# fxzjshm/simple-radio-telescope-backend

Hardware: AMD Instinct MI355X
Metric: baseband Msamples/sec/node + real-time ratio, J1644-4559 config at 1/2/4/8 MI355X (higher is better)
Workload: dtype fp32; 1 GPU; model=J1644-4559 coherent-dedispersion single-pulse pipeline, baseband_input_count=1073741824, nsamps_reserved=23494656, baseband_input_bits=2, spectrum_channel_count=2048, rfi=True, phase_table=False, fft_backend=native, parallelism=stream-sharded dp1, global_batch=1, seq_len=1073741824

## Files before the change

csrc/bind/module.cpp:

```cpp

#include <torch/extension.h>
#include <pybind11/numpy.h>
#include <ATen/cuda/CUDAContext.h>
#include <c10/cuda/CUDAGuard.h>

#include <functional>
#include <vector>

#include "../engine/engine.h"
#include "../fft/native_fft.h"
#include "../include/srtb_kernels.h"

namespace {

using namespace srtb_hip;

hipStream_t cur_stream() {
  return at::cuda::getCurrentCUDAStream().stream();
}

void check(hipError_t e, const char* what) { check_hip(e, what); }

#define CHECK_CUDA(t) TORCH_CHECK((t).is_cuda(), #t " must be on GPU")
#define CHECK_CONTIG(t) TORCH_CHECK((t).is_contiguous(), #t " must be contiguous")
// ... 627 lines not shown
  auto out = torch::empty({nc}, torch::TensorOptions()
                                    .dtype(torch::kComplexFloat)
                                    .device(dev));
  check(dedisp_poly_factors(cptr(out), (size_t)nc, (uint32_t)n,
                            (size_t)stride, f_min, f_c, df, dm, cur_stream()),
        "dedisp_poly_factors");
  return out;
}

torch::Tensor t_native_rfft(torch::Tensor x) {
  CHECK_CUDA(x);
  CHECK_CONTIG(x);
  TORCH_CHECK(x.scalar_type() == torch::kFloat32);
  const size_t n = x.numel();
  const size_t m = n / 2;
  auto stream = cur_stream();
  NativeFft plan;
  plan.plan(m, 1, -1, stream);
  auto z = torch::empty({(int64_t)m},
                        x.options().dtype(torch::kComplexFloat));
  auto packed = x.view({(int64_t)m, 2});
  auto work = torch::empty_like(z);
  work.copy_(torch::view_as_complex(packed));
  plan.exec(cptr(work), cptr(z), stream);
  check(r2c_post_process(cptr(z), cptr(z), m, nullptr, nullptr, stream),
        "r2c post");
  check(hipStreamSynchronize(stream), "native_rfft sync");
  return z;
}


double time_iters(hipStream_t stream, int iters, const std::function<void()>& f) {
  hipEvent_t e0, e1;
  check(hipEventCreate(&e0), "ev");
  check(hipEventCreate(&e1), "ev");
  f();
  check(hipStreamSynchronize(stream), "warm sync");
  check(hipEventRecord(e0, stream), "rec");
  for (int i = 0; i < iters; ++i) f();
  check(hipEventRecord(e1, stream), "rec");
  check(hipEventSynchronize(e1), "sync");
  float ms = 0;
  check(hipEventElapsedTime(&ms, e0, e1), "elapsed");
  hipEventDestroy(e0);
  hipEventDestroy(e1);
  return ms / iters;
}

double t_bench_fft(int64_t len, int64_t batch, int64_t sign, int64_t iters,
                   std::string backend) {
  auto stream = cur_stream();
// ... 20 lines not shown
    ms = time_iters(stream, (int)iters, [&] {
      hipfftExecC2C(h, reinterpret_cast<hipfftComplex*>(xp),
                    reinterpret_cast<hipfftComplex*>(yp),
                    sign < 0 ? HIPFFT_FORWARD : HIPFFT_BACKWARD);
    });
    hipfftDestroy(h);
  }
  return ms;
}

double t_bench_rfft(int64_t n, int64_t iters, std::string backend) {
  auto stream = cur_stream();
  auto x = torch::randn({n}, torch::TensorOptions()
                                 .dtype(torch::kFloat32)
                                 .device(torch::kCUDA));
  auto y = torch::empty({n / 2 + 1, 2}, x.options());
  float* xp = x.data_ptr<float>();
  float2* yp = reinterpret_cast<float2*>(y.data_ptr());
  double ms = 0;
  if (backend == "native") {
    const size_t m = n / 2;
    NativeFft plan;
    plan.plan(m, 1, -1, stream);
    ms = time_iters(stream, (int)iters, [&] {
      plan.exec(reinterpret_cast<float2*>(xp), yp, stream);
      check(r2c_post_process(yp, yp, m, nullptr, nullptr, stream), "post");
    });
  } else {
    hipfftHandle h;
    check_fft(hipfftCreate(&h), "create");
    long long n1[1] = {(long long)n};
    size_t ws = 0;
    check_fft(hipfftMakePlanMany64(h, 1, n1, nullptr, 1, 0, nullptr, 1, 0,
                                   HIPFFT_R2C, 1, &ws),
              "plan");
    check_fft(hipfftSetStream(h, stream), "stream");
    ms = time_iters(stream, (int)iters, [&] {
      hipfftExecR2C(h, xp, reinterpret_cast<hipfftComplex*>(yp));
    });
    hipfftDestroy(h);
  }
  return ms;
}


class PyEngine {
 public:
  PyEngine(int64_t n, int64_t nbits, int64_t channels, double freq_low,
           double bandwidth, double sample_rate, double dm,
// ... 310 lines not shown
  m.def("subtract_mean", &t_subtract_mean);
  m.def("count_signal", &t_count_signal);
  m.def("inclusive_scan", &t_inclusive_scan);
  m.def("boxcar", &t_boxcar);
  m.def("boxcar_ladder", &t_boxcar_ladder, py::arg("cumsum"),
        py::arg("lengths"), py::arg("snr"));
  m.def("resample_power", &t_resample_power);
  m.def("normalize_by_mean", &t_normalize_by_mean);
  m.def("generate_pixmap", &t_generate_pixmap);
  m.def("running_mean", &t_running_mean);
  m.def("correlate", &t_correlate);
  m.def("filterbank_detect", &t_filterbank_detect, py::arg("wf"),
        py::arg("flags"), py::arg("valid_rows"), py::arg("tscrunch"),
        py::arg("fscrunch"), py::arg("reverse"));
  m.def("filterbank_channel_stats", &t_filterbank_channel_stats, py::arg("P"));
  m.def("filterbank_quantize", &t_filterbank_quantize, py::arg("P"),
        py::arg("mean"), py::arg("std"));
  m.def("fold_block", &t_fold_block, py::arg("wf"), py::arg("flags"),
        py::arg("valid"), py::arg("nbin"), py::arg("phi"), py::arg("dphi"),
        py::arg("acc"), py::arg("hits"), py::arg("weights"));
  m.def("native_fft", &t_native_fft, py::arg("x"), py::arg("sign"));
  m.def("native_fft_sk", &t_native_fft_sk, py::arg("x"));
  m.def("native_rfft", &t_native_rfft, py::arg("x"));
  m.def("preop_backward_fft", &t_preop_backward_fft, py::arg("spec"),
        py::arg("maxcol_log2"), py::arg("final_log2"), py::arg("f_min"),
        py::arg("f_c"), py::arg("df"), py::arg("dms"),
        py::arg("ranges") = std::vector<std::vector<int64_t>>{},
        py::arg("enable_rfi") = false, py::arg("threshold") = 0.0,
        py::arg("channel_count") = 1);
  m.def("dedisp_poly_factors", &t_dedisp_poly_factors);
  m.def("bench_fft", &t_bench_fft, py::arg("len"), py::arg("batch"),
        py::arg("sign"), py::arg("iters") = 20, py::arg("backend") = "native");
  m.def("bench_rfft", &t_bench_rfft, py::arg("n"), py::arg("iters") = 20,
        py::arg("backend") = "native");

  py::class_<PyEngine>(m, "PipelineEngine")
      .def(py::init<int64_t, int64_t, int64_t, double, double, double, double,
                    double, double, double, int64_t, int64_t,
                    std::vector<std::vector<int64_t>>, bool, bool, bool,
                    int64_t, int64_t, int64_t, bool, int64_t, int64_t,
                    int64_t, int64_t, int64_t, double, double, double>(),
           py::arg("n"), py::arg("nbits"), py::arg("channels"),
           py::arg("freq_low"), py::arg("bandwidth"), py::arg("sample_rate"),
           py::arg("dm"), py::arg("rfi_threshold") = 10.0,
           py::arg("sk_threshold") = 1.1, py::arg("snr_threshold") = 6.0,
           py::arg("max_boxcar") = 1024, py::arg("nsamps_reserved") = 0,
// ... 49 lines not shown
```

csrc/engine/engine.cpp:

```cpp
#include "engine.h"

#include <roctracer/roctx.h>

#include <algorithm>
#include <cmath>
#include <cstdlib>
#include <cstring>
#include <stdexcept>
#include <string>

namespace srtb_hip {

namespace {
constexpr double kD = 4.148808e3;

uint64_t fold_turns_to_word(double x) {
  const double v = std::ldexp(x, 64);
  if (v >= 0x1p64) return 0;
  if (v >= 0x1p63) return (uint64_t)v;
  return (uint64_t)std::llrint(v);
}

struct RoctxRange {
  bool on;
// ... 207 lines not shown
      check_hip(hipMalloc(&s.fold_table,
                          fold_table_words(fold_v_) * sizeof(uint32_t)),
                "fold table alloc");
      check_hip(hipHostMalloc(&s.h_fold_words, 2 * sizeof(uint64_t)),
                "pinned fold words");
      check_hip(hipMemset(s.fold_acc, 0, s_ * nb * sizeof(double)),
                "fold acc clear");
      check_hip(hipMemset(s.fold_hits, 0, nb * sizeof(uint64_t)),
                "fold hits clear");
      check_hip(hipMemset(s.fold_weights, 0, s_ * sizeof(uint64_t)),
                "fold weights clear");
      check_hip(hipDeviceSynchronize(), "fold clear sync");
    }
    fused_unpack_off_ = std::getenv("SRTB_NO_FUSED_UNPACK") != nullptr;
    if (const char* sc = std::getenv("SRTB_SERIAL_CHAINS"))
      serial_chains_ = std::atoi(sc) != 0 ? 1 : 0;
    const int be = cfg.fft_backend;
    native_fft_ = (be == 0 || be == 2) && NativeFft::supported(nc_);
    native_bwd_ = native_fft_ && NativeFft::supported(l_) &&
                  (be == 0 || l_ >= (1ull << 17));
    fuse_r2c_ = false;
    if (native_fft_) {
      s.nfwd.plan(nc_, 1, -1, s.stream);
      if (native_bwd_) {
        const char* b32 = std::getenv("SRTB_FFT_BWD32");
        if (b32 && std::atoi(b32) != 0)
          s.nbwd.plan(l_, s_, +1, s.stream, 5,
                      8);
        else
          s.nbwd.plan(l_, s_, +1, s.stream);
        const int wpr = s.nbwd.dif_sk_wgs_per_row();
        if (cfg.enable_sk && wpr > 0 && cfg.window_kind == 0)
          check_hip(hipMalloc(&s.sk_dif_partials,
                              s_ * (size_t)wpr * sizeof(float2)),
                    "sk dif partials");
      } else {
        s.plans.create_c2c_only(l_, s_, s.stream);
      }
      check_hip(hipStreamSynchronize(s.stream), "fft table sync");
      {
        const char* fe = std::getenv("SRTB_FUSE_R2C");
        const bool want = fe && std::atoi(fe) != 0;
        const int fwgs = s.nfwd.dif_sk_wgs_per_row();
        fuse_r2c_ = want && native_bwd_ && s.nbwd.first_pass_fusable() &&
                    fwgs > 0;
        if (fuse_r2c_) {
// ... 22 lines not shown
  if (cfg.use_phase_table) {
    check_hip(hipMalloc(&phase_table_, nc_ * sizeof(float2)), "table alloc");
    check_hip(dedisp_phase_table(phase_table_, nc_, f_min_, f_c_, df_, cfg.dm,
                                 slots_[0]->stream),
              "phase table");
    check_hip(hipStreamSynchronize(slots_[0]->stream), "table sync");
  }
}

PipelineEngine::~PipelineEngine() {
  for (auto& sp : slots_) {
    if (sp->stream) (void)hipStreamSynchronize(sp->stream);
  }
  for (auto& sp : slots_) {
    Slot& s = *sp;
    s.plans.destroy();
    (void)hipFree(s.raw);
    (void)hipFree(s.samples);
    (void)hipFree(s.spec);
    (void)hipFree(s.s2s4);
    if (s.sk_dif_partials) (void)hipFree(s.sk_dif_partials);
    if (s.xbuf) (void)hipFree(s.xbuf);
    if (s.fwd_pw) (void)hipFree(s.fwd_pw);
    (void)hipFree(s.flags);
    (void)hipFree(s.ts);
    (void)hipFree(s.ts_partial);
    (void)hipFree(s.cumsum);
    (void)hipFree(s.box);
    (void)hipFree(s.scan_scratch);
    (void)hipFree(s.partials);
    if (s.box_partials) (void)hipFree(s.box_partials);
    (void)hipFree(s.mean_power);
    (void)hipFree(s.sums);
    (void)hipFree(s.counters);
    (void)hipFree(s.thresholds);
    (void)hipHostFree(s.h_counters);
    (void)hipHostFree(s.h_thresholds);
    if (s.trial_w) {
      (void)hipFree(s.trial_w);
      (void)hipFree(s.trial_plane);
      (void)hipFree(s.trial_counters);
      (void)hipFree(s.trial_thresholds);
      (void)hipFree(s.trial_peak_val);
      (void)hipFree(s.trial_peak_idx);
      (void)hipHostFree(s.h_trial_counters);
      (void)hipHostFree(s.h_trial_thresholds);
// ... 208 lines not shown
                           (in_bits == 1 || in_bits == 2 || in_bits == 4 ||
                            in_bits == 8 || in_bits == -8 ||
                            in_bits == 16 || in_bits == -16) &&
                           !window_ && slots_[0]->nfwd.first_pass_fusable();
  if (dev_raw && !fuse_unpack) {
    check_hip(unpack(dev_raw, s.samples, n_, cfg_.baseband_input_bits,
                     window_, st),
              "unpack");
  } else if (!dev_raw && native_fft_) {
    check_hip(hipMemcpyAsync(s.samples, dev_samples, n_ * sizeof(float),
                             hipMemcpyDeviceToDevice, st),
              "samples d2d");
  } else if (!dev_raw) {
    fft_in = dev_samples;
  }
  if (native_fft_ && fr2c) {
    s.nfwd.exec(reinterpret_cast<float2*>(s.samples), s.spec, st,
                nullptr, cfg_.enable_rfi_s1 ? s.fwd_pw : nullptr,
                fuse_unpack ? dev_raw : nullptr, in_bits);
    if (cfg_.enable_rfi_s1)
      check_hip(r2c_mean_from_power(s.fwd_pw, fwd_pw_n_, s.spec, nc_,
                                    s.mean_power, st),
                "r2c mean");
  } else if (native_fft_) {
    s.nfwd.exec(reinterpret_cast<float2*>(s.samples), s.spec, st,
                nullptr, nullptr, fuse_unpack ? dev_raw : nullptr, in_bits);
    check_hip(r2c_post_process(
                  s.spec, s.spec, nc_,
                  cfg_.enable_rfi_s1 ? s.partials : nullptr,
                  cfg_.enable_rfi_s1 ? s.mean_power : nullptr, st),
              "r2c post");
  } else {
    s.plans.exec_r2c(const_cast<float*>(fft_in), s.spec);
    if (cfg_.enable_rfi_s1)
      check_hip(mean_power(s.spec, nc_, s.partials, s.mean_power, st),
                "meanp");
  }
}

void PipelineEngine::enqueue_back(Slot& s, double dm, const ResultRow& row,
                                  float* ts_dst, bool keep_spectrum) {
  hipStream_t st = s.stream;
  const float2* table = phase_table_;
  const bool fr2c = fuse_r2c_;
  const bool fuse_into_bwd = native_bwd_ && s.nbwd.first_pass_fusable();
  const FftPreop pre = make_preop(s, dm);
// ... 429 lines not shown
```

csrc/engine/engine.h:

```cpp

#pragma once

#include <hip/hip_runtime.h>

#include <array>
#include <cstdint>
#include <memory>
#include <vector>

#include "../fft/fft_plans.h"
#include "../fft/native_fft.h"
#include "../include/srtb_kernels.h"

namespace srtb_hip {

struct EngineConfig {
  size_t baseband_input_count = 1ull << 28;
  int baseband_input_bits = 8;
  size_t spectrum_channel_count = 1ull << 15;
  double freq_low = 1000.0;
  double bandwidth = 500.0;
  double sample_rate = 1e9;
  double dm = 0.0;
  float rfi_threshold = 10.0f;
// ... 158 lines not shown
  int n_slots_ = 2;

  float2* phase_table_ = nullptr;
  float* window_ = nullptr;
  float* watfft_window_ = nullptr;
  bool native_fft_ = false;
  bool fused_unpack_off_ = false;
  bool native_bwd_ = false;
  bool fuse_r2c_ = false;
  size_t fwd_pw_n_ = 0;


  struct Slot {
    hipStream_t stream = nullptr;
    hipEvent_t done = nullptr;
    bool busy = false;
    bool wf_zap_pending = false;
    float2* wf = nullptr;
    uint8_t* raw = nullptr;
    float* samples = nullptr;
    float2* spec = nullptr;
    float2* xbuf = nullptr;
    float2* fwd_pw = nullptr;
    float2* s2s4 = nullptr;
    float2* sk_dif_partials = nullptr;
    uint8_t* flags = nullptr;
    float* ts = nullptr;
    float* ts_partial = nullptr;
    float* cumsum = nullptr;
    float* box = nullptr;
    float* scan_scratch = nullptr;
    double* partials = nullptr;
    double* box_partials = nullptr;
    double* mean_power = nullptr;
    double* sums = nullptr;
    unsigned* counters = nullptr;
    float* thresholds = nullptr;
    unsigned* h_counters = nullptr;
    float* h_thresholds = nullptr;
    FftPlanSet plans;
    NativeFft nfwd, nbwd;
    hipGraphExec_t graph_exec = nullptr;
    const void* graph_host_src = nullptr;
    int graph_pending = 0;
    float2* trial_w = nullptr;
    float* trial_plane = nullptr;
// ... 34 lines not shown
```

csrc/fft/native_fft.h:

```cpp

#pragma once

#include <algorithm>
#include <cstdint>
#include <cstdlib>
#include <cmath>
#include <stdexcept>
#include <string>
#include <vector>

#include "../include/srtb_kernels.h"
#include "fft_plans.h"

namespace srtb_hip {

class NativeFft {
 public:
  static constexpr uint32_t kMaxPassLen = 4096;
  static int elems_per_wg() {
    const char* e = std::getenv("SRTB_FFT_ELEMS");
    int v = e ? std::atoi(e) : 4096;
    if (v < 512) v = 512;
    if (v > 8192) v = 8192;
    return v;
  }

  static bool is_pow2(size_t v) { return v && (v & (v - 1)) == 0; }

  static bool supported(size_t len) {
    return is_pow2(len) && len >= 2 &&
           len <= (size_t)kMaxPassLen * kMaxPassLen * kMaxPassLen;
  }

  NativeFft() = default;
  NativeFft(const NativeFft&) = delete;
  NativeFft& operator=(const NativeFft&) = delete;
  ~NativeFft() { destroy(); }

  void plan(size_t len, size_t batch, int sign, hipStream_t stream,
            int maxcol_log2_ovr = 0, int final_log2_ovr = 0) {
    destroy();
    if (!supported(len)) throw std::runtime_error("NativeFft: unsupported len");
    len_ = len;
    batch_ = batch;
    sign_ = sign;

    const size_t L = len;
    const int t = ilog2z(len);
    passes_.clear();
    if (t <= 12) {
      const char* we = std::getenv("SRTB_FFT_WAVE");
      const int wv = we ? std::atoi(we) : 1;
      if (t >= 8 && t <= 11 && wv != 0) {
        ensure_len_table((uint32_t)len, sign, stream);
        Pass p;
        p.kind = PassKind::kWave;
        p.d.n = (uint32_t)len;
        p.n_ffts = batch;
        p.tw_n = len_table((uint32_t)len);
        passes_.push_back(p);
        return;
      }
      if (t == 12 && !std::getenv("SRTB_FFT_NOSP_DIF")) {
        ensure_len_table((uint32_t)len, sign, stream);
        Pass p;
        p.kind = PassKind::kDif;
        p.d.n = (uint32_t)len;
        p.dif.n = (uint32_t)len;
// ... 99 lines not shown
      p.n_ffts = batch * (L / f[j]);
      p.tw_n = len_table(f[j]);
      p.tw_hi = mod_hi(M[j]);
      p.tw_lo = mod_lo(M[j]);
      passes_.push_back(p);
    }
    {
      const uint32_t fn = f[m - 1];
      ensure_len_table(fn, sign, stream);
      Pass p;
      p.kind = PassKind::kDif;
      p.d.n = fn;
      p.dif.n = fn;
      p.dif.out_c2 = L;
      p.dif.out_elem_coef = Cp[m - 1];
      p.dif.n_prefix = m - 1;
      for (int w = 0; w < m - 1; ++w) {
        p.dif.pf_bits[w] = ilog2z(f[w]);
        p.dif.pf_coef[w] = M[w + 1] / fn;
      }
      p.n_ffts = batch * (L / fn);
      p.tw_n = len_table(fn);
      passes_.push_back(p);
    }
  }

  int n_passes() const { return (int)passes_.size(); }

  bool first_pass_fusable() const {
    return !passes_.empty() && passes_[0].kind == PassKind::kCol;
  }

  bool preop_uses_poly(const FftPreop& preop) const {
    return first_pass_fusable() &&
           fft_col_preop_uses_poly(passes_[0].d, passes_[0].n_ffts, sign_,
                                   preop);
  }

  int dif_sk_wgs_per_row() const {
    if (passes_.empty() || passes_.back().kind != PassKind::kDif) return 0;
    const Pass& p = passes_.back();
    const size_t per_row = (len_ / p.dif.n);
    const int F = dif_f(p);
    if (per_row % F != 0) return 0;
    return (int)(per_row / F);
  }

  void exec(const float2* in, float2* out, hipStream_t stream,
            const FftPreop* preop = nullptr,
            float2* dif_sk_partials = nullptr,
            const uint8_t* decode2_raw = nullptr, int decode_bits = 2,
            float2* first_pass_out = nullptr) {
    if (passes_.empty()) throw std::runtime_error("NativeFft: not planned");
    if (passes_.size() > 1 && in == out && !first_pass_out)
      throw std::runtime_error("NativeFft: multi-pass needs out != in");
    if (preop && preop->r2c_m && !first_pass_out)
      throw std::runtime_error("NativeFft: r2c fusion needs first_pass_out");
    if (preop && !first_pass_fusable())
      throw std::runtime_error("NativeFft: preop needs a column first pass");
    if (decode2_raw && (preop || !first_pass_fusable()))
      throw std::runtime_error("NativeFft: decode2 needs a column first pass");
    float2* cur = const_cast<float2*>(in);
    for (size_t i = 0; i < passes_.size(); ++i) {
      Pass& p = passes_[i];
      const bool last = (i + 1 == passes_.size());
      float2* dst = last ? out : cur;
      const FftPreop* pre = (i == 0) ? preop : nullptr;
      switch (p.kind) {
        case PassKind::kStockham: {
          const int F = pick_f(p.d.n, p, p.n_ffts);
          check_hip(fft_stockham_pass(cur, dst, p.d, p.n_ffts, F,
                                      p.load_ffast, p.store_ffast, sign_,
                                      p.tw_n, p.tw_hi, p.tw_lo, stream),
                    "fft_stockham_pass");
          break;
        }
        case PassKind::kCol: {
          float2* o = (i == 0 && first_pass_out) ? first_pass_out : cur;
          check_hip(fft_col_pass(cur, o, p.d, p.n_ffts, sign_, p.tw_n,
                                 p.tw_hi, p.tw_lo, stream, pre,
                                 i == 0 ? decode2_raw : nullptr, decode_bits),
                    "fft_col_pass");
          dst = o;
          break;
        }
        case PassKind::kMid:
          check_hip(fft_mid512_pass(cur, cur, p.d, p.n_ffts, sign_, p.tw_n,
                                    stream),
                    "fft_mid512_pass");
          dst = cur;
          break;
        case PassKind::kWave:
          check_hip(fft_wave_pass(cur, dst, p.d.n, p.n_ffts, sign_, p.tw_n,
                                  stream),
                    "fft_wave_pass");
          break;
        case PassKind::kDif: {
          const int F = dif_f(p);
          check_hip(fft_dif_final(cur, dst, p.dif, p.n_ffts, F, sign_,
                                  p.tw_n, dif_sk_partials, stream),
                    "fft_dif_final");
          break;
        }
      }
      cur = dst;
    }
  }

  void destroy() {
    for (auto& t : tables_) (void)hipFree(t.ptr);
    tables_.clear();
    passes_.clear();
  }

 private:
  enum class PassKind { kStockham, kCol, kMid, kDif, kWave };

  struct Pass {
    PassKind kind = PassKind::kStockham;
    FftPassDesc d{};
// ... 8 lines not shown
  struct Table {
    int kind;
    size_t key;
    float2* ptr;
  };

  static int ilog2z(size_t v) {
    int t = 0;
    while ((1ull << t) < v) ++t;
    return t;
  }

  int dif_f(const Pass& p) const {
    int F = (p.dif.n <= 64) ? 32 : 16;
    if (const char* e = std::getenv("SRTB_FFT_DIF_F")) {
      const int v = std::atoi(e);
      if (v >= 1 && v <= 64 && (v & (v - 1)) == 0) F = v;
    }
    while (F > 1 &&
           ((size_t)p.dif.n + (size_t)F * (p.dif.n + 2)) * sizeof(float2) >
               80 * 1024)
      F >>= 1;
    while (F > 1 && p.n_ffts % F != 0) F >>= 1;
    return F;
  }

  int pick_f(uint32_t n, const Pass& p, size_t n_ffts) const {
    size_t f = (size_t)elems_per_wg() / n;
    if (f < 1) f = 1;
    while (f > 1 &&
           ((size_t)n + 2ull * f * (n + 2) + 16) * sizeof(float2) >
               160 * 1024)
      f >>= 1;
    while (f > 1 && n_ffts % f != 0) f >>= 1;
    if (p.d.d0 > 1 && f > p.d.d0) f = p.d.d0;
    while (f > 1 && n_ffts % f != 0) f >>= 1;
    return (int)f;
  }

  void ensure_len_table(uint32_t n, int sign, hipStream_t stream) {
    if (len_table(n)) return;
    float2* t = nullptr;
    check_hip(hipMalloc(&t, std::max<size_t>(n, 1) * sizeof(float2)),
              "tw_n alloc");
    check_hip(fft_build_twiddle(t, std::max<size_t>(n, 1), (double)n, sign,
                                stream),
// ... 22 lines not shown
    tables_.push_back({1, mod, thi});
    tables_.push_back({2, mod, tlo});
  }

  float2* len_table(uint32_t n) const {
    for (auto& t : tables_)
      if (t.kind == 0 && t.key == n) return t.ptr;
    return nullptr;
  }
  float2* mod_hi(size_t mod) const {
    for (auto& t : tables_)
      if (t.kind == 1 && t.key == mod) return t.ptr;
    return nullptr;
  }
  float2* mod_lo(size_t mod) const {
    for (auto& t : tables_)
      if (t.kind == 2 && t.key == mod) return t.ptr;
    return nullptr;
  }
  int mod_lo_bits(size_t mod) const { return mod_lo_bits_for(mod); }

  size_t len_ = 0, batch_ = 0;
  int sign_ = -1;
  std::vector<Pass> passes_;
  std::vector<Table> tables_;
};

}
```

csrc/include/srtb_kernels.h:

```cpp

#pragma once

#include <hip/hip_runtime.h>
#include <cstddef>
#include <cstdint>

namespace srtb_hip {

hipError_t unpack(const uint8_t* in, float* out, size_t out_count, int nbits,
                  const float* window, hipStream_t stream);

hipError_t unpack_interleaved_2pol(const int8_t* in, float* out0, float* out1,
                                   size_t count_per_pol, const float* window,
                                   hipStream_t stream);

hipError_t unpack_naocpsr_snap1(const int8_t* in, float* out0, float* out1,
                                size_t count_per_pol, const float* window,
                                hipStream_t stream);

hipError_t unpack_gznupsr_a1(const uint8_t* in, float* out0, float* out1,
                             float* out2, float* out3, int n_streams,
                             size_t count_per_stream, const float* window,
                             hipStream_t stream);

// ... 164 lines not shown
bool fft_col_preop_uses_poly(const FftPassDesc& d, size_t n_ffts, int sign,
                             const FftPreop& preop);

hipError_t dedisp_poly_factors(float2* out, size_t nc, uint32_t n,
                               size_t stride, double f_min, double f_c,
                               double df, double dm, hipStream_t stream);

struct DifFinalDesc {
  uint32_t n;
  unsigned long long out_c2;
  unsigned long long out_elem_coef;
  int n_prefix = 0;
  int pf_bits[4] = {0, 0, 0, 0};
  unsigned long long pf_coef[4] = {0, 0, 0, 0};
};
hipError_t fft_mid512_pass(const float2* in, float2* out,
                           const FftPassDesc& d, size_t n_ffts, int sign,
                           const float2* tw_n, hipStream_t stream);

hipError_t fft_dif_final(const float2* in, float2* out, const DifFinalDesc& d,
                         size_t n_ffts, int F, int sign, const float2* tw_n,
                         float2* sk_partials, hipStream_t stream);

hipError_t sk_combine_partials(const float2* partials, size_t rows,
                               int wgs_per_row, float2* s2s4,
                               hipStream_t stream);

hipError_t r2c_post_process(const float2* z, float2* x, size_t m,
                            double* mean_partials, double* out_mean,
                            hipStream_t stream);

hipError_t resample_power_2d(const float2* wf, size_t rows, size_t len,
                             float* out, int out_h, int out_w,
                             hipStream_t stream);

hipError_t normalize_by_mean(float* img, size_t n, const double* sum,
                             hipStream_t stream);

hipError_t generate_pixmap(const float* intensity, uint32_t* out, size_t n,
                           uint32_t color0, uint32_t color1,
                           uint32_t color_overflow, hipStream_t stream);

hipError_t running_mean_init(const float* data, size_t nsamp, size_t nchan,
                             size_t windowsize, float* ave, hipStream_t stream);
hipError_t running_mean(const float* data, size_t nsamp, size_t nchan,
                        uint8_t* out, size_t windowsize, float* ave,
// ... 11 lines not shown
```

csrc/kernels/fft.hip:

```cpp

#include <cmath>
#include <cstdlib>
#include "common.h"
#include "../include/srtb_kernels.h"

namespace srtb_hip {

namespace {

__device__ inline float2 cmulf(float2 a, float2 b) {
  return make_float2(a.x * b.x - a.y * b.y, a.x * b.y + a.y * b.x);
}

}

struct FftPassDescDev {
  uint32_t n;
  int n_log2, f_log2;
  int d0_log2, d1_log2;
  unsigned long long in_c0, in_c1, in_c2;
  unsigned long long in_stride;
  unsigned long long out_c0, out_c1, out_c2;
  unsigned long long out_stride;
  unsigned long long tw_f0, tw_f1;
// ... 1023 lines not shown
    }
    __syncthreads();
  }

  {
    const int f = threadIdx.x & (F - 1);
    unsigned long long q0, q1, q2;
    digits(col0 + f, d, q0, q1, q2);
    const bool active = (col0 + f) < n_ffts;
    constexpr int TPC = 256 / F;
    for (int r = 0; r < 512 / TPC; ++r) {
      const int k = r * TPC + (threadIdx.x >> LOGF);
      const unsigned rk = rev4_bits((unsigned)(k >> 1), 8);
      const float2 v = X[f * LDST + 256 * (k & 1) + dif_swz((int)rk)];
      float2 rr = v;
      const unsigned long long m_ =
          (q0 * d.tw_f0 * (unsigned long long)k) & d.tw_mask;
      rr = cmulf(rr, tw_eval(m_, d.tw_angle));
      if (active) out[base_f + (uint32_t)k * stride32] = rr;
    }
  }
}

template <bool MEANP>
__global__ void k_r2c_post(const float2* __restrict__ z,
                           float2* __restrict__ x, size_t m,
                           double* __restrict__ partials) {
  const size_t stride = (size_t)gridDim.x * blockDim.x;
  const size_t half = m / 2;
  double acc = 0.0;
  for (size_t k = (size_t)blockIdx.x * blockDim.x + threadIdx.x; k <= half;
       k += stride) {
    const float2 zk = z[k];
    const float2 zm = z[k == 0 ? 0 : m - k];
    const float2 zmc = make_float2(zm.x, -zm.y);
    const float2 even = make_float2(0.5f * (zk.x + zmc.x),
                                    0.5f * (zk.y + zmc.y));
    const float2 dif = make_float2(zk.x - zmc.x, zk.y - zmc.y);
    const float2 odd = make_float2(0.5f * dif.y, -0.5f * dif.x);
    const float phiw = (float)(-M_PI * (double)k / (double)m);
    float sw, cw;
    __sincosf(phiw, &sw, &cw);
    const float2 w = make_float2(cw, sw);
    const float2 wo = cmulf(w, odd);
    const float2 xk = make_float2(even.x + wo.x, even.y + wo.y);
    x[k] = xk;
    if constexpr (MEANP) acc += (double)xk.x * xk.x + (double)xk.y * xk.y;
    if (k != 0 && k != half) {
      const float2 xm = make_float2(even.x - wo.x, -(even.y - wo.y));
      x[m - k] = xm;
      if constexpr (MEANP)
        acc += (double)xm.x * xm.x + (double)xm.y * xm.y;
    }
  }
  if constexpr (MEANP) {
    const double b = block_reduce_sum(acc);
    if (threadIdx.x == 0) partials[blockIdx.x] = b;
  }
}

__global__ void k_r2c_post_finish_mean(const double* __restrict__ partials,
                                       int np, size_t n,
                                       double* __restrict__ out_mean) {
  double acc = 0.0;
  for (int i = threadIdx.x; i < np; i += blockDim.x) acc += partials[i];
  const double b = block_reduce_sum(acc);
  if (threadIdx.x == 0) *out_mean = b / (double)n;
}

constexpr int kR2cPostBlocks = 1024;

inline int ilog2(unsigned long long v) {
  int t = 0;
  while ((1ull << t) < v) ++t;
  return t;
}

}

hipError_t fft_build_twiddle(float2* table, size_t count, double m, int sign,
                             hipStream_t stream) {
  hipLaunchKernelGGL(k_build_twiddle, grid_for(count), dim3(kBlock), 0,
                     stream, table, count, sign * 2.0 * M_PI / m);
  SRTB_CHECK_LAUNCH();
  return hipSuccess;
}

static bool use_pair32() {
  static const bool v = [] {
    const char* e = std::getenv("SRTB_FFT_PAIR32");
// ... 506 lines not shown
    wgs_per_row = (int)(per_row / F);
  }
  if (sign < 0) {
    if (sk_partials)
      hipLaunchKernelGGL((k_fft_dif_final<-1, true>), dim3(grid), dim3(256),
                         lds_bytes, stream, in, out, d, tw_n, sk_partials,
                         wgs_per_row);
    else
      hipLaunchKernelGGL((k_fft_dif_final<-1, false>), dim3(grid), dim3(256),
                         lds_bytes, stream, in, out, d, tw_n, nullptr, 0);
  } else {
    if (sk_partials)
      hipLaunchKernelGGL((k_fft_dif_final<1, true>), dim3(grid), dim3(256),
                         lds_bytes, stream, in, out, d, tw_n, sk_partials,
                         wgs_per_row);
    else
      hipLaunchKernelGGL((k_fft_dif_final<1, false>), dim3(grid), dim3(256),
                         lds_bytes, stream, in, out, d, tw_n, nullptr, 0);
  }
  SRTB_CHECK_LAUNCH();
  return hipSuccess;
}

hipError_t sk_combine_partials(const float2* partials, size_t rows,
                               int wgs_per_row, float2* s2s4,
                               hipStream_t stream) {
  hipLaunchKernelGGL(k_sk_combine_partials, grid_for(rows), dim3(kBlock), 0,
                     stream, partials, rows, wgs_per_row, s2s4);
  SRTB_CHECK_LAUNCH();
  return hipSuccess;
}

hipError_t r2c_post_process(const float2* z, float2* x, size_t m,
                            double* mean_partials, double* out_mean,
                            hipStream_t stream) {
  if (mean_partials) {
    hipLaunchKernelGGL((k_r2c_post<true>), dim3(kR2cPostBlocks), dim3(kBlock),
                       0, stream, z, x, m, mean_partials);
    hipLaunchKernelGGL(k_r2c_post_finish_mean, dim3(1), dim3(kBlock), 0,
                       stream, mean_partials, kR2cPostBlocks, m, out_mean);
  } else {
    hipLaunchKernelGGL((k_r2c_post<false>), dim3(kR2cPostBlocks), dim3(kBlock),
                       0, stream, z, x, m, nullptr);
  }
  SRTB_CHECK_LAUNCH();
  return hipSuccess;
// ... 4 lines not shown
```

srtb_amd/fftref.py:

```python

from __future__ import annotations

import numpy as np


def bit_reverse_indices(n: int) -> np.ndarray:
    t = n.bit_length() - 1
    idx = np.arange(n)
    rev = np.zeros(n, dtype=np.int64)
    for b in range(t):
        rev |= ((idx >> b) & 1) << (t - 1 - b)
    return rev


def twiddle_table(n: int, sign: int) -> np.ndarray:
    j = np.arange(n // 2)
    return np.exp(sign * 2j * np.pi * j / n).astype(np.complex64)


def fft_small(x: np.ndarray, sign: int, dtype=np.complex64) -> np.ndarray:
    n = x.size
    assert n & (n - 1) == 0
    tw = twiddle_table(n, sign).astype(np.complex128)
    y = np.asarray(x, dtype=np.complex128)[bit_reverse_indices(n)].copy()
# ... 111 lines not shown
    for n2 in range(l2):
        col = fft1(m[:, n2])
        k1 = np.arange(l1)
        col = col * np.exp(sign * 2j * np.pi * (k1 * n2) / n)
        m[:, n2] = col
    out = np.empty(n, dtype=np.complex128)
    for k1 in range(l1):
        row = fft2(m[k1, :])
        out[k1 + l1 * np.arange(l2)] = row
    return out.astype(np.complex64)


def fft_deep(x: np.ndarray, factors: list[int], sign: int) -> np.ndarray:
    if len(factors) == 1:
        return fft_small(x, sign, np.complex128).astype(np.complex64)
    l1 = factors[0]
    l2 = int(np.prod(factors[1:]))
    return fft_four_step(
        x, l1, l2, sign,
        fft1=lambda v: fft_small(v, sign, np.complex128),
        fft2=lambda v: fft_deep(v, factors[1:], sign).astype(np.complex128))


def r2c_post(z: np.ndarray, sign: int = -1) -> np.ndarray:
    m = z.size
    zf = np.asarray(z, dtype=np.complex128)
    zk = zf
    zmk = np.conj(np.roll(zf[::-1], 1))
    k = np.arange(m)
    w = np.exp(sign * 2j * np.pi * k / (2 * m))
    even = 0.5 * (zk + zmk)
    odd = -0.5j * (zk - zmk)
    return (even + w * odd).astype(np.complex64)


def rfft_packed(x: np.ndarray, factors: list[int] | None = None) -> np.ndarray:
    x = np.asarray(x, dtype=np.float64)
    n = x.size
    z = x[0::2] + 1j * x[1::2]
    if factors is None:
        zf = np.fft.fft(z)
    else:
        zf = fft_deep(z.astype(np.complex64), factors, -1).astype(np.complex128)
    return r2c_post(zf, -1)


def plan_factors(t: int, maxcol_log2: int = 6, final_log2: int | None = None) -> list[int]:
    if t <= 12:
        return [1 << t]
    if final_log2 is None:
        final_log2 = 6 if t >= 14 else 8
    if final_log2 % 2:
        final_log2 += 1
    final_log2 = min(max(final_log2, 6), 12)
    if final_log2 >= t:
        final_log2 = t - 1 if t % 2 else t - 2
# ... 19 lines not shown
```

Before: 65860 Msamples/s.

## Fuse real-to-complex post-processing into final DIF FFT pass with mirrored-row pairing

```diff
diff --git a/csrc/bind/module.cpp b/csrc/bind/module.cpp
--- a/csrc/bind/module.cpp
+++ b/csrc/bind/module.cpp
@@ -673,11 +673,25 @@
   auto packed = x.view({(int64_t)m, 2});
   auto work = torch::empty_like(z);
   work.copy_(torch::view_as_complex(packed));
-  plan.exec(cptr(work), cptr(z), stream);
-  check(r2c_post_process(cptr(z), cptr(z), m, nullptr, nullptr, stream),
-        "r2c post");
+  if (plan.r2c_final_partials()) {
+    const NativeFft::R2cFinal rf;
+    plan.exec(cptr(work), cptr(z), stream, nullptr, nullptr, nullptr, 2,
+              nullptr, &rf);
+  } else {
+    plan.exec(cptr(work), cptr(z), stream);
+    check(r2c_post_process(cptr(z), cptr(z), m, nullptr, nullptr, stream),
+          "r2c post");
+  }
   check(hipStreamSynchronize(stream), "native_rfft sync");
   return z;
+}
+
+int64_t t_native_rfft_final_partials(int64_t n) {
+  auto stream = cur_stream();
+  NativeFft plan;
+  plan.plan((size_t)n / 2, 1, -1, stream);
+  check(hipStreamSynchronize(stream), "native_rfft plan sync");
+  return plan.r2c_final_partials();
 }
 
 
@@ -744,9 +758,16 @@
     const size_t m = n / 2;
     NativeFft plan;
     plan.plan(m, 1, -1, stream);
+    const bool fused = plan.r2c_final_partials() != 0;
+    const NativeFft::R2cFinal rf;
     ms = time_iters(stream, (int)iters, [&] {
-      plan.exec(reinterpret_cast<float2*>(xp), yp, stream);
-      check(r2c_post_process(yp, yp, m, nullptr, nullptr, stream), "post");
+      if (fused) {
+        plan.exec(reinterpret_cast<float2*>(xp), yp, stream, nullptr, nullptr,
+                  nullptr, 2, nullptr, &rf);
+      } else {
+        plan.exec(reinterpret_cast<float2*>(xp), yp, stream);
+        check(r2c_post_process(yp, yp, m, nullptr, nullptr, stream), "post");
+      }
     });
   } else {
     hipfftHandle h;
@@ -1103,6 +1124,8 @@
   m.def("native_fft", &t_native_fft, py::arg("x"), py::arg("sign"));
   m.def("native_fft_sk", &t_native_fft_sk, py::arg("x"));
   m.def("native_rfft", &t_native_rfft, py::arg("x"));
+  m.def("native_rfft_final_partials", &t_native_rfft_final_partials,
+        py::arg("n"));
   m.def("preop_backward_fft", &t_preop_backward_fft, py::arg("spec"),
         py::arg("maxcol_log2"), py::arg("final_log2"), py::arg("f_min"),
         py::arg("f_c"), py::arg("df"), py::arg("dms"),
diff --git a/csrc/engine/engine.cpp b/csrc/engine/engine.cpp
--- a/csrc/engine/engine.cpp
+++ b/csrc/engine/engine.cpp
@@ -253,6 +253,9 @@
     fuse_r2c_ = false;
     if (native_fft_) {
       s.nfwd.plan(nc_, 1, -1, s.stream);
+      if (const int rp = s.nfwd.r2c_final_partials())
+        check_hip(hipMalloc(&s.r2c_final_partials, rp * sizeof(double)),
+                  "r2c final partials alloc");
       if (native_bwd_) {
         const char* b32 = std::getenv("SRTB_FFT_BWD32");
         if (b32 && std::atoi(b32) != 0)
@@ -321,6 +324,7 @@
     if (s.sk_dif_partials) (void)hipFree(s.sk_dif_partials);
     if (s.xbuf) (void)hipFree(s.xbuf);
     if (s.fwd_pw) (void)hipFree(s.fwd_pw);
+    if (s.r2c_final_partials) (void)hipFree(s.r2c_final_partials);
     (void)hipFree(s.flags);
     (void)hipFree(s.ts);
     (void)hipFree(s.ts_partial);
@@ -575,6 +579,15 @@
       check_hip(r2c_mean_from_power(s.fwd_pw, fwd_pw_n_, s.spec, nc_,
                                     s.mean_power, st),
                 "r2c mean");
+  } else if (native_fft_ && s.r2c_final_partials) {
+    NativeFft::R2cFinal rf;
+    if (cfg_.enable_rfi_s1) {
+      rf.mean_partials = s.r2c_final_partials;
+      rf.out_mean = s.mean_power;
+    }
+    s.nfwd.exec(reinterpret_cast<float2*>(s.samples), s.spec, st, nullptr,
+                nullptr, fuse_unpack ? dev_raw : nullptr, in_bits, nullptr,
+                &rf);
   } else if (native_fft_) {
     s.nfwd.exec(reinterpret_cast<float2*>(s.samples), s.spec, st,
                 nullptr, nullptr, fuse_unpack ? dev_raw : nullptr, in_bits);
diff --git a/csrc/engine/engine.h b/csrc/engine/engine.h
--- a/csrc/engine/engine.h
+++ b/csrc/engine/engine.h
@@ -204,6 +204,7 @@
     float2* spec = nullptr;
     float2* xbuf = nullptr;
     float2* fwd_pw = nullptr;
+    double* r2c_final_partials = nullptr;
     float2* s2s4 = nullptr;
     float2* sk_dif_partials = nullptr;
     uint8_t* flags = nullptr;
diff --git a/csrc/fft/native_fft.h b/csrc/fft/native_fft.h
--- a/csrc/fft/native_fft.h
+++ b/csrc/fft/native_fft.h
@@ -44,6 +44,9 @@
     len_ = len;
     batch_ = batch;
     sign_ = sign;
+    const char* rf = std::getenv("SRTB_FFT_R2C_FINAL");
+    r2c_final_ = !(rf && std::atoi(rf) == 0);
+    r2c_f_ = 0;
 
     const size_t L = len;
     const int t = ilog2z(len);
@@ -189,6 +192,7 @@
       p.n_ffts = batch * (L / fn);
       p.tw_n = len_table(fn);
       passes_.push_back(p);
+      r2c_f_ = dif_r2c_f(p);
     }
   }
 
@@ -213,12 +217,28 @@
     return (int)(per_row / F);
   }
 
+  int r2c_final_partials() const {
+    if (!r2c_final_ || sign_ != -1 || batch_ != 1 || passes_.size() < 2 ||
+        passes_.back().kind != PassKind::kDif)
+      return 0;
+    const Pass& p = passes_.back();
+    return fft_dif_final_r2c_wgs(p.n_ffts, r2c_f_);
+  }
+
+  struct R2cFinal {
+    double* mean_partials = nullptr;
+    double* out_mean = nullptr;
+  };
+
   void exec(const float2* in, float2* out, hipStream_t stream,
             const FftPreop* preop = nullptr,
             float2* dif_sk_partials = nullptr,
             const uint8_t* decode2_raw = nullptr, int decode_bits = 2,
-            float2* first_pass_out = nullptr) {
+            float2* first_pass_out = nullptr,
+            const R2cFinal* r2c_final = nullptr) {
     if (passes_.empty()) throw std::runtime_error("NativeFft: not planned");
+    if (r2c_final && (r2c_final_partials() == 0 || dif_sk_partials))
+      throw std::runtime_error("NativeFft: r2c final-pass fusion n/a");
     if (passes_.size() > 1 && in == out && !first_pass_out)
       throw std::runtime_error("NativeFft: multi-pass needs out != in");
     if (preop && preop->r2c_m && !first_pass_out)
@@ -263,6 +283,14 @@
                     "fft_wave_pass");
           break;
         case PassKind::kDif: {
+          if (last && r2c_final) {
+            check_hip(fft_dif_final_r2c(cur, dst, p.dif, p.n_ffts,
+                                        r2c_f_, p.tw_n,
+                                        r2c_final->mean_partials,
+                                        r2c_final->out_mean, stream),
+                      "fft_dif_final_r2c");
+            break;
+          }
           const int F = dif_f(p);
           check_hip(fft_dif_final(cur, dst, p.dif, p.n_ffts, F, sign_,
                                   p.tw_n, dif_sk_partials, stream),
@@ -317,6 +345,22 @@
                80 * 1024)
       F >>= 1;
     while (F > 1 && p.n_ffts % F != 0) F >>= 1;
+    return F;
+  }
+
+  int dif_r2c_f(const Pass& p) const {
+    int F = (p.dif.n <= 64) ? 32 : 16;
+    for (const char* name : {"SRTB_FFT_DIF_F", "SRTB_FFT_R2C_F"}) {
+      if (const char* e = std::getenv(name)) {
+        const int v = std::atoi(e);
+        if (v >= 1 && v <= 64 && (v & (v - 1)) == 0) F = v;
+      }
+    }
+    while (F > 1 &&
+           ((size_t)p.dif.n + 2 * (size_t)F * (p.dif.n + 2)) * sizeof(float2) >
+               80 * 1024)
+      F >>= 1;
+    while (F > 1 && p.n_ffts % (2 * (size_t)F) != 0) F >>= 1;
     return F;
   }
 
@@ -385,6 +429,8 @@
 
   size_t len_ = 0, batch_ = 0;
   int sign_ = -1;
+  bool r2c_final_ = true;
+  int r2c_f_ = 0;
   std::vector<Pass> passes_;
   std::vector<Table> tables_;
 };
diff --git a/csrc/include/srtb_kernels.h b/csrc/include/srtb_kernels.h
--- a/csrc/include/srtb_kernels.h
+++ b/csrc/include/srtb_kernels.h
@@ -210,6 +210,12 @@
                          size_t n_ffts, int F, int sign, const float2* tw_n,
                          float2* sk_partials, hipStream_t stream);
 
+int fft_dif_final_r2c_wgs(size_t n_ffts, int F);
+hipError_t fft_dif_final_r2c(const float2* in, float2* out,
+                             const DifFinalDesc& d, size_t n_ffts, int F,
+                             const float2* tw_n, double* mean_partials,
+                             double* out_mean, hipStream_t stream);
+
 hipError_t sk_combine_partials(const float2* partials, size_t rows,
                                int wgs_per_row, float2* s2s4,
                                hipStream_t stream);
diff --git a/csrc/kernels/fft.hip b/csrc/kernels/fft.hip
--- a/csrc/kernels/fft.hip
+++ b/csrc/kernels/fft.hip
@@ -1069,6 +1069,22 @@
   }
 }
 
+__device__ __forceinline__ void r2c_pair_combine(float2 zk, float2 zm,
+                                                 float phiw, float2& xk,
+                                                 float2& xm) {
+  const float2 zmc = make_float2(zm.x, -zm.y);
+  const float2 even = make_float2(0.5f * (zk.x + zmc.x),
+                                  0.5f * (zk.y + zmc.y));
+  const float2 dif = make_float2(zk.x - zmc.x, zk.y - zmc.y);
+  const float2 odd = make_float2(0.5f * dif.y, -0.5f * dif.x);
+  float sw, cw;
+  __sincosf(phiw, &sw, &cw);
+  const float2 wo = make_float2(__builtin_fmaf(cw, odd.x, -(sw * odd.y)),
+                                __builtin_fmaf(cw, odd.y, sw * odd.x));
+  xk = make_float2(even.x + wo.x, even.y + wo.y);
+  xm = make_float2(even.x - wo.x, -(even.y - wo.y));
+}
+
 template <bool MEANP>
 __global__ void k_r2c_post(const float2* __restrict__ z,
                            float2* __restrict__ x, size_t m,
@@ -1080,21 +1096,12 @@
        k += stride) {
     const float2 zk = z[k];
     const float2 zm = z[k == 0 ? 0 : m - k];
-    const float2 zmc = make_float2(zm.x, -zm.y);
-    const float2 even = make_float2(0.5f * (zk.x + zmc.x),
-                                    0.5f * (zk.y + zmc.y));
-    const float2 dif = make_float2(zk.x - zmc.x, zk.y - zmc.y);
-    const float2 odd = make_float2(0.5f * dif.y, -0.5f * dif.x);
     const float phiw = (float)(-M_PI * (double)k / (double)m);
-    float sw, cw;
-    __sincosf(phiw, &sw, &cw);
-    const float2 w = make_float2(cw, sw);
-    const float2 wo = cmulf(w, odd);
-    const float2 xk = make_float2(even.x + wo.x, even.y + wo.y);
+    float2 xk, xm;
+    r2c_pair_combine(zk, zm, phiw, xk, xm);
     x[k] = xk;
     if constexpr (MEANP) acc += (double)xk.x * xk.x + (double)xk.y * xk.y;
     if (k != 0 && k != half) {
-      const float2 xm = make_float2(even.x - wo.x, -(even.y - wo.y));
       x[m - k] = xm;
       if constexpr (MEANP)
         acc += (double)xm.x * xm.x + (double)xm.y * xm.y;
@@ -1113,6 +1120,173 @@
   for (int i = threadIdx.x; i < np; i += blockDim.x) acc += partials[i];
   const double b = block_reduce_sum(acc);
   if (threadIdx.x == 0) *out_mean = b / (double)n;
+}
+
+template <bool MEANP>
+__global__ void __launch_bounds__(256)
+    k_fft_dif_final_r2c(const float2* __restrict__ in,
+                        float2* __restrict__ out, DifFinalDescDev d,
+                        const float2* __restrict__ tw_n,
+                        double* __restrict__ partials, uint32_t tuning) {
+  extern __shared__ float2 lds[];
+  const int n = d.n;
+  const int nl = d.n_log2;
+  const int F = 1 << d.f_log2;
+  const int ldst = n + 2;
+  float2* ltw = lds;
+  float2* X = lds + n;
+  const unsigned long long P = 1ull << d.j_bits;
+  const unsigned long long m = d.row_len;
+  const bool row0 = blockIdx.x == gridDim.x - 1;
+  const int rows = row0 ? 1 : 2 * F;
+  const unsigned int w =
+      row0 ? blockIdx.x : xcd_swizzle(blockIdx.x, gridDim.x - 1, tuning);
+  const unsigned long long j0 =
+      ((unsigned long long)w << d.f_log2) + 1;
+  const int total = rows << nl;
+
+  for (int j = threadIdx.x; j < n; j += blockDim.x) ltw[j] = tw_n[j];
+
+  auto instance_of = [&](int r) -> unsigned long long {
+    if (row0) return 0;
+    return r < F ? j0 + r : P - (j0 + (r - F));
+  };
+  {
+    const int iters = total >> 8;
+    int it = 0;
+    for (; it + 8 <= iters; it += 8) {
+      float2 tmp[8];
+      int lidx[8];
+#pragma unroll
+      for (int k = 0; k < 8; ++k) {
+        const int e = ((it + k) << 8) + threadIdx.x;
+        const int r = e >> nl;
+        const int i = e & (n - 1);
+        unsigned long long in_blk, obase;
+        dif_addr(instance_of(r), d, in_blk, obase);
+        tmp[k] = in[in_blk + i];
+        lidx[k] = r * ldst + dif_swz(i);
+      }
+#pragma unroll
+      for (int k = 0; k < 8; ++k) X[lidx[k]] = tmp[k];
+    }
+    for (int e = (it << 8) + threadIdx.x; e < total; e += blockDim.x) {
+      const int r = e >> nl;
+      const int i = e & (n - 1);
+      unsigned long long in_blk, obase;
+      dif_addr(instance_of(r), d, in_blk, obase);
+      X[r * ldst + dif_swz(i)] = in[in_blk + i];
+    }
+  }
+  __syncthreads();
+
+  const int quarter = n >> 2;
+  for (int L = n, tl = 0; L >= 4; L >>= 2, tl += 2) {
+    const int M = L >> 2;
+    const int m_log2 = (nl - tl) - 2;
+    for (int b = threadIdx.x; b < rows * quarter; b += blockDim.x) {
+      const int r = b >> (nl - 2);
+      const int bb = b & (quarter - 1);
+      const int j = bb & (M - 1);
+      const int g = (bb >> m_log2) << (m_log2 + 2);
+      float2* row = X + r * ldst;
+      const int e0 = dif_swz(g + j);
+      const int e1 = dif_swz(g + j + M);
+      const int e2 = dif_swz(g + j + 2 * M);
+      const int e3 = dif_swz(g + j + 3 * M);
+      const float2 a = row[e0];
+      const float2 bv = row[e1];
+      const float2 c = row[e2];
+      const float2 dv = row[e3];
+      const float2 t0 = make_float2(a.x + c.x, a.y + c.y);
+      const float2 t1 = make_float2(a.x - c.x, a.y - c.y);
+      const float2 t2 = make_float2(bv.x + dv.x, bv.y + dv.y);
+      const float2 dmy = make_float2(bv.x - dv.x, bv.y - dv.y);
+      const float2 t3 = make_float2(dmy.y, -dmy.x);
+      const float2 x0 = make_float2(t0.x + t2.x, t0.y + t2.y);
+      const float2 x1 = make_float2(t1.x + t3.x, t1.y + t3.y);
+      const float2 x2 = make_float2(t0.x - t2.x, t0.y - t2.y);
+      const float2 x3 = make_float2(t1.x - t3.x, t1.y - t3.y);
+      const int ts = tl;
+      row[e0] = x0;
+      row[e1] = (j == 0) ? x1 : cmulf(x1, ltw[(j << ts)]);
+      row[e2] = (j == 0) ? x2 : cmulf(x2, ltw[(2 * j) << ts]);
+      row[e3] = (j == 0) ? x3 : cmulf(x3, ltw[(3 * j) << ts]);
+    }
+    __syncthreads();
+  }
+
+  const double inv_m = 1.0 / (double)m;
+  const int half_n = n >> 1;
+  double acc = 0.0;
+  if (!row0) {
+    for (int e = threadIdx.x; e < (F << nl); e += blockDim.x) {
+      const int f = e & (F - 1);
+      const int k = e >> d.f_log2;
+      const unsigned long long J = j0 + f;
+      const bool low = k < half_n;
+      if (J == (P >> 1) && !low) continue;
+      const unsigned rk = rev4_bits((unsigned)k, nl);
+      const float2 own = X[f * ldst + dif_swz((int)rk)];
+      const float2 mir =
+          X[(F + f) * ldst + dif_swz((int)(rk ^ (unsigned)(n - 1)))];
+      const unsigned long long ko =
+          low ? J + (unsigned long long)k * P
+              : (P - J) + (unsigned long long)(n - 1 - k) * P;
+      const float phiw = (float)(-M_PI * (double)ko * inv_m);
+      float2 xk, xm;
+      r2c_pair_combine(low ? own : mir, low ? mir : own, phiw, xk, xm);
+      out[ko] = xk;
+      out[m - ko] = xm;
+      if constexpr (MEANP) {
+        acc += (double)xk.x * xk.x + (double)xk.y * xk.y;
+        acc += (double)xm.x * xm.x + (double)xm.y * xm.y;
+      }
+    }
+  } else {
+    for (int k = threadIdx.x; k <= half_n; k += blockDim.x) {
+      const float2 zk = X[dif_swz((int)rev4_bits((unsigned)k, nl))];
+      const float2 zm =
+          X[dif_swz((int)rev4_bits((unsigned)(k == 0 ? 0 : n - k), nl))];
+      const unsigned long long ko = (unsigned long long)k * P;
+      const float phiw = (float)(-M_PI * (double)ko * inv_m);
+      float2 xk, xm;
+      r2c_pair_combine(zk, zm, phiw, xk, xm);
+      out[ko] = xk;
+      if constexpr (MEANP) acc += (double)xk.x * xk.x + (double)xk.y * xk.y;
+      if (k != 0 && k != half_n) {
+        out[m - ko] = xm;
+        if constexpr (MEANP)
+          acc += (double)xm.x * xm.x + (double)xm.y * xm.y;
+      }
+    }
+  }
+  if constexpr (MEANP) {
+    const double b = block_reduce_sum(acc);
+    if (threadIdx.x == 0) partials[row0 ? blockIdx.x : w] = b;
+  }
+}
+
+__global__ void __launch_bounds__(1024)
+    k_r2c_final_finish_mean(const double* __restrict__ partials, int np,
+                            size_t n, double* __restrict__ out_mean) {
+  __shared__ double wsum[1024 / 64];
+  double a[8] = {0.0, 0.0, 0.0, 0.0, 0.0, 0.0, 0.0, 0.0};
+  int i = threadIdx.x;
+  for (; i + 7 * 1024 < np; i += 8 * 1024) {
+#pragma unroll
+    for (int u = 0; u < 8; ++u) a[u] += partials[i + u * 1024];
+  }
+  for (; i < np; i += 1024) a[0] += partials[i];
+  const double acc = wave_reduce_sum(((a[0] + a[1]) + (a[2] + a[3])) +
+                                     ((a[4] + a[5]) + (a[6] + a[7])));
+  if ((threadIdx.x & 63) == 0) wsum[threadIdx.x >> 6] = acc;
+  __syncthreads();
+  if (threadIdx.x == 0) {
+    double t = 0.0;
+    for (int k = 0; k < 1024 / 64; ++k) t += wsum[k];
+    *out_mean = t / (double)n;
+  }
 }
 
 constexpr int kR2cPostBlocks = 1024;
@@ -1665,6 +1839,58 @@
   return hipSuccess;
 }
 
+int fft_dif_final_r2c_wgs(size_t n_ffts, int F) {
+  if (F < 1 || n_ffts < 2 * (size_t)F || n_ffts % (2 * (size_t)F) != 0)
+    return 0;
+  return (int)(n_ffts / (2 * (size_t)F)) + 1;
+}
+
+hipError_t fft_dif_final_r2c(const float2* in, float2* out,
+                             const DifFinalDesc& hd, size_t n_ffts, int F,
+                             const float2* tw_n, double* mean_partials,
+                             double* out_mean, hipStream_t stream) {
+  if (hd.n & (hd.n - 1)) return hipErrorInvalidValue;
+  if (in == out || hd.n_prefix < 1) return hipErrorInvalidValue;
+  DifFinalDescDev d;
+  d.n = hd.n;
+  d.n_log2 = ilog2(hd.n);
+  if (d.n_log2 & 1) return hipErrorInvalidValue;
+  if (F & (F - 1)) return hipErrorInvalidValue;
+  d.f_log2 = ilog2((unsigned)F);
+  d.row_len = hd.out_c2;
+  d.out_elem_coef = hd.out_elem_coef;
+  d.n_prefix = hd.n_prefix;
+  int jb = 0;
+  for (int i = 0; i < 4; ++i) {
+    d.pf_bits[i] = hd.pf_bits[i];
+    d.pf_coef[i] = hd.pf_coef[i];
+    if (i < hd.n_prefix) jb += hd.pf_bits[i];
+  }
+  d.j_bits = jb;
+  if (n_ffts != (1ull << jb) || n_ffts * hd.n != hd.out_c2)
+    return hipErrorInvalidValue;
+  const int grid = fft_dif_final_r2c_wgs(n_ffts, F);
+  if (grid == 0) return hipErrorInvalidValue;
+  const size_t lds_bytes =
+      ((size_t)hd.n + 2 * (size_t)F * (hd.n + 2)) * sizeof(float2);
+  if (lds_bytes > 160 * 1024) return hipErrorInvalidValue;
+  const char* xe = std::getenv("SRTB_FFT_R2C_XCD");
+  const uint32_t tuning = (xe && std::atoi(xe) == 0) ? 0u : 1u;
+  if (mean_partials) {
+    hipLaunchKernelGGL((k_fft_dif_final_r2c<true>), dim3(grid), dim3(256),
+                       lds_bytes, stream, in, out, d, tw_n, mean_partials,
+                       tuning);
+    hipLaunchKernelGGL(k_r2c_final_finish_mean, dim3(1), dim3(1024), 0,
+                       stream, mean_partials, grid, (size_t)hd.out_c2,
+                       out_mean);
+  } else {
+    hipLaunchKernelGGL((k_fft_dif_final_r2c<false>), dim3(grid), dim3(256),
+                       lds_bytes, stream, in, out, d, tw_n, nullptr, tuning);
+  }
+  SRTB_CHECK_LAUNCH();
+  return hipSuccess;
+}
+
 hipError_t sk_combine_partials(const float2* partials, size_t rows,
                                int wgs_per_row, float2* s2s4,
                                hipStream_t stream) {
diff --git a/srtb_amd/fftref.py b/srtb_amd/fftref.py
--- a/srtb_amd/fftref.py
+++ b/srtb_amd/fftref.py
@@ -157,7 +157,7 @@
         fft2=lambda v: fft_deep(v, factors[1:], sign).astype(np.complex128))
 
 
-def r2c_post(z: np.ndarray, sign: int = -1) -> np.ndarray:
+def r2c_post(z: np.ndarray, sign: int = -1, dtype=np.complex64) -> np.ndarray:
     m = z.size
     zf = np.asarray(z, dtype=np.complex128)
     zk = zf
@@ -166,7 +166,57 @@
     w = np.exp(sign * 2j * np.pi * k / (2 * m))
     even = 0.5 * (zk + zmk)
     odd = -0.5j * (zk - zmk)
-    return (even + w * odd).astype(np.complex64)
+    return (even + w * odd).astype(dtype)
+
+
+def r2c_final_store(p: int, n: int, f: int) -> dict[str, np.ndarray]:
+    assert p >= 2 * f and p % (2 * f) == 0 and n % 2 == 0
+    half = n // 2
+    rec: dict[str, list] = {key: [] for key in (
+        "wg", "row", "k", "prow", "pk", "inst", "pinst", "ko", "pair")}
+
+    def emit(**cols):
+        size = max(np.size(v) for v in cols.values())
+        for key, v in cols.items():
+            rec[key].append(np.broadcast_to(np.asarray(v, np.int64), (size,)))
+
+    kk = np.arange(n)
+    low = kk < half
+    for w in range(p // (2 * f)):
+        for r in range(f):
+            j = w * f + 1 + r
+            sel = low if j == p // 2 else np.ones(n, bool)
+            k = kk[sel]
+            lo = low[sel]
+            emit(wg=w,
+                 row=np.where(lo, r, f + r), k=np.where(lo, k, n - 1 - k),
+                 prow=np.where(lo, f + r, r), pk=np.where(lo, n - 1 - k, k),
+                 inst=np.where(lo, j, p - j), pinst=np.where(lo, p - j, j),
+                 ko=np.where(lo, j + k * p, (p - j) + (n - 1 - k) * p),
+                 pair=1)
+    k = np.arange(half + 1)
+    emit(wg=p // (2 * f), row=0, k=k, prow=0, pk=np.where(k == 0, 0, n - k),
+         inst=0, pinst=0, ko=k * p, pair=(k != 0) & (k != half))
+    return {key: np.concatenate(v) for key, v in rec.items()}
+
+
+def r2c_final_spectrum(z: np.ndarray, n: int, f: int) -> np.ndarray:
+    m = z.size
+    p = m // n
+    s = r2c_final_store(p, n, f)
+    zf = np.asarray(z, dtype=np.complex128)
+    w = np.exp(-2j * np.pi * np.arange(m) / (2 * m))
+
+    def combine(a, b, idx):
+        return 0.5 * (a + np.conj(b)) + w[idx] * (-0.5j * (a - np.conj(b)))
+
+    zk = zf[s["inst"] + s["k"] * p]
+    zm = zf[s["pinst"] + s["pk"] * p]
+    out = np.full(m, np.nan + 1j * np.nan, dtype=np.complex128)
+    out[s["ko"]] = combine(zk, zm, s["ko"])
+    pair = s["pair"] == 1
+    out[m - s["ko"][pair]] = combine(zm[pair], zk[pair], m - s["ko"][pair])
+    return out
 
 
 def rfft_packed(x: np.ndarray, factors: list[int] | None = None) -> np.ndarray:
```

New measurement: 71390 Msamples/s (median of 6 runs). +8.4%, better.
